# facebookresearch/CPC_audio

Hardware: AMD Instinct MI355X
Metric: audio-seconds/sec (train step) (higher is better)
Workload: dtype f32 (conv GEMMs and the GRU forward recurrence: fp32 operands as 2 scaled fp16 pieces -- the inputs of conv1/conv2 stored that way --, 3 fp16 MFMAs per product; GRU backward recurrence and the criterion's dz gather-GEMM: f32 MFMAs; InfoNCE scores: 2 fp16 pieces; other GEMMs: 3 bf16 pieces, 6 bf16 MF

## Files before the change

cpc_audio_amd/_lib.py:

```python
import ctypes
import os
import threading

_HERE = os.path.dirname(os.path.abspath(__file__))
LIB_PATH = os.path.join(_HERE, "lib", "libcpc_hip.so")
DEFAULT_GRU_MODE = 2
DEFAULT_GRU_XCD_LOCAL = 1
DEFAULT_GRU_POLL_PLAIN = 15
DEFAULT_MFMA_MODE = 3
EXPECTED_ABI = 16
DEFAULT_DMA_PIPELINE = 2
DEFAULT_WGRAD_DMA_STAGES = 4
DEFAULT_CONV_SMALL_PIPE = 1
DEFAULT_GRU_WGRAD_STREAM = 1
DEFAULT_NCE_FUSED = 2
DEFAULT_INDEX_PREP_GROUPS = -1
DEFAULT_FWD_NSPLIT = 0
DEFAULT_DGRAD_NSPLIT = 256
DEFAULT_STEP_SCHEDULE = (1, 0)

_P = ctypes.c_void_p
_I = ctypes.c_int
_L = ctypes.c_long
_F = ctypes.c_float

SIGNATURES = {
    "cpc_abi_version": (_I, []),
    "cpc_release_stream": (_I, [_P]),
    "cpc_streams_overlap": (_I, [_P, _P, _P]),
    "cpc_set_mfma_mode": (_I, [_I]),
    "cpc_get_mfma_mode": (_I, []),
    "cpc_device_error_flags": (_I, [_I]),
    "cpc_conv0_forward": (_I, [_P] * 8 + [_I, _I, _P]),
    "cpc_conv0_forward_h2": (_I, [_P] * 9 + [_I, _I, _P]),
    "cpc_h2_encode": (_I, [_P, _P, _L, _P, _P]),
    "cpc_h2_decode": (_I, [_P, _P, _L, _P, _P]),
    "cpc_conv_weight_relayout_h2": (_I, [_P, _P, _I, _P]),
    "cpc_conv_gemm_forward_h2": (_I, [_P] * 11 + [_I] * 6 + [_P]),
    "cpc_set_dma_tile": (_I, [_I]),
    "cpc_set_conv0_tuning": (_I, [_I, _I]),
# ... 216 lines not shown
```

cpc_audio_amd/csrc/gru.hip:

```cpp
#include "cpc_common.h"
#include "cpc_internal.h"
#include "gemm_tile.h"
#include "persist.h"

namespace cpc {

constexpr int kH = kC;
constexpr int kG = 3 * kH;

__global__ __launch_bounds__(256) void gru_step_fwd_kernel(
    const float* __restrict__ hprev, long hp_bstride, const float* __restrict__ whh,
    const float* __restrict__ bhh, const float* __restrict__ gi, float* __restrict__ y,
    float* __restrict__ Rg, float* __restrict__ Zg, float* __restrict__ Ng, float* __restrict__ GHN,
    float* __restrict__ hN, int B, int S, int t) {
    __shared__ float part[4][3][256];
    const int tid = threadIdx.x, lane = tid & 63, w = tid >> 6;
    const int i = lane & 15, kq = lane >> 4;
    const int j0 = blockIdx.x * 16, b0 = blockIdx.y * 16;
    const int koff = 64 * w + 4 * kq;

    float4 a[4];
    {
        const bool ok = hprev != nullptr && (b0 + i) < B;
        const float* ap = hprev + (ok ? (long)(b0 + i) * hp_bstride + koff : 0);
// ... 218 lines not shown
    if (layer == 0) {
#pragma unroll
        for (int g = 0; g < 3; ++g)
            gh[g] = (((part[0][g][e] + part[1][g][e]) + (part[2][g][e] + part[3][g][e])) +
                     ((part[4][g][e] + part[5][g][e]) + (part[6][g][e] + part[7][g][e]))) + bh[g];
    } else {
#pragma unroll
        for (int g = 0; g < 3; ++g)
            gh[g] = ((part[0][g][e] + part[1][g][e]) + (part[2][g][e] + part[3][g][e])) + bh[g];
        gi_r += (part[4][0][e] + part[5][0][e]) + (part[6][0][e] + part[7][0][e]);
        gi_z += (part[4][1][e] + part[5][1][e]) + (part[6][1][e] + part[7][1][e]);
        gi_n += (part[4][2][e] + part[5][2][e]) + (part[6][2][e] + part[7][2][e]);
    }
    const float r = sigmoidf_(gi_r + gh[0]);
    const float z = sigmoidf_(gi_z + gh[1]);
    const float n = tanhf(gi_n + r * gh[2]);
    const float h = (1.0f - z) * n + z * hp;
    p.y[layer][bt * kH + j] = h;
    p.R[layer][bt * kH + j] = r;
    p.Z[layer][bt * kH + j] = z;
    p.N[layer][bt * kH + j] = n;
    p.GHN[layer][bt * kH + j] = gh[2];
    if (t == S - 1) p.hN[((long)layer * B + b) * kH + j] = h;
}

struct Gru2Bwd {
    const float* dy;
    const float* whhT[2];
    const float* wih1T;
    const float* Z[2];
    const float* cr[2]; const float* cz[2]; const float* cnh[2]; const float* cni[2];
    float* dGi[2]; float* dGh[2]; float* DH[2];
    float* xdh[2];
    int B, S;
    int spin_limit;
    int ntiles, xcd_pack;
    int tile0, total_tiles;
    int first_sleep;
    int poll_plain;
    unsigned* xsync;
};

__global__ __launch_bounds__(256) void gru_bwd_coef_kernel(
    const float* __restrict__ R, const float* __restrict__ Z, const float* __restrict__ N,
    const float* __restrict__ GHN, const float* __restrict__ y, const float* __restrict__ h0,
    float* __restrict__ cr, float* __restrict__ cz, float* __restrict__ cnh, float* __restrict__ cni, int B, int S) {
    const int ntiles = (B + 15) >> 4;
    const long idx = (long)blockIdx.x * 256 + threadIdx.x;
    if (idx >= (long)ntiles * 16 * S * 64) return;
    const int u4 = (int)(idx & 63);
    const long bt = idx >> 6;
    const int b = (int)(bt / S), t = (int)(bt - (long)b * S);
    const long dst = xtile(t, b >> 4, ntiles, kH) + xpos(b & 15, 4 * u4);
    if (b >= B) {
        const float4 zero = make_float4(0.f, 0.f, 0.f, 0.f);
        *reinterpret_cast<float4*>(cr + dst) = zero;
        *reinterpret_cast<float4*>(cz + dst) = zero;
        *reinterpret_cast<float4*>(cnh + dst) = zero;
        *reinterpret_cast<float4*>(cni + dst) = zero;
        return;
    }
    const long src = bt * kH + 4 * u4;
    const float4 r = *reinterpret_cast<const float4*>(R + src), z = *reinterpret_cast<const float4*>(Z + src);
    const float4 n = *reinterpret_cast<const float4*>(N + src), g = *reinterpret_cast<const float4*>(GHN + src);
    float4 hp = make_float4(0.f, 0.f, 0.f, 0.f);
    if (t > 0) hp = *reinterpret_cast<const float4*>(y + src - kH);
// ... 77 lines not shown
        }
    } else if (w < 4) {
        if (has_next) {
            const float* grow = p.dGh[0] + (bok ? ((long)(b0 + i) * S + t + 1) * kG : 0);
            acc = mfma_gate_rows<4>(acc, grow, bok, p.whhT[0] + (long)(j0 + i) * kG, 64 * w + 4 * kq);
        }
    } else {
        const float* grow = p.dGi[1] + (bok ? ((long)(b0 + i) * S + t) * kG : 0);
        acc = mfma_gate_rows<4>(acc, grow, bok, p.wih1T + (long)(j0 + i) * kG, 64 * (w - 4) + 4 * kq);
    }
#pragma unroll
    for (int rr = 0; rr < 4; ++rr) part[w][(kq * 4 + rr) * 16 + i] = acc[rr];
    __syncthreads();
    if (!gate_thread) return;
    const int e = tid;
    const float dh = (((part[0][e] + part[1][e]) + (part[2][e] + part[3][e])) +
                      ((part[4][e] + part[5][e]) + (part[6][e] + part[7][e]))) + dh0;
    float* gi = p.dGi[layer] + bt * kG;
    float* gh = p.dGh[layer] + bt * kG;
    const float dar = dh * cr, daz = dh * cz;
    gi[j] = dar;            gh[j] = dar;
    gi[kH + j] = daz;       gh[kH + j] = daz;
    gi[2 * kH + j] = dh * cni;   gh[2 * kH + j] = dh * cnh;
    p.DH[layer][bt * kH + j] = dh;
}

constexpr int kSpinLimit = 1 << 20;
static __device__ unsigned g_gru_poll_timeout = 0;

__device__ __forceinline__ void store_handover(float* p, float v, bool local) {
    if (local) __hip_atomic_store(p, v, __ATOMIC_RELAXED, __HIP_MEMORY_SCOPE_WAVEFRONT);
    else __hip_atomic_store(p, v, __ATOMIC_RELAXED, __HIP_MEMORY_SCOPE_AGENT);
}
__device__ __forceinline__ bool tile_on_one_xcd(unsigned* sync, int spin_limit) {
    __shared__ unsigned verdict;
    if (threadIdx.x == 0) {
        const unsigned xid = __builtin_amdgcn_s_getreg((3 << 11) | 20) & 15u;
        __hip_atomic_fetch_and(sync, ~(1u << xid), __ATOMIC_RELAXED, __HIP_MEMORY_SCOPE_AGENT);
        __hip_atomic_fetch_add(sync + 1, 1u, __ATOMIC_RELEASE, __HIP_MEMORY_SCOPE_AGENT);
        int budget = spin_limit < 4096 ? spin_limit : 4096;
        while (__hip_atomic_load(sync + 1, __ATOMIC_ACQUIRE, __HIP_MEMORY_SCOPE_AGENT) != 31u && budget-- > 0) __builtin_amdgcn_s_sleep(8);
        const unsigned gone = ~__hip_atomic_load(sync, __ATOMIC_RELAXED, __HIP_MEMORY_SCOPE_AGENT);
        verdict = (budget > 0 && gone != 0u && (gone & (gone - 1u)) == 0u) ? 1u : 0u;
    }
    __syncthreads();
    return verdict != 0u;
}

template <int NII>
__device__ __forceinline__ void poll_row(const float* __restrict__ row, bool ok, float4 (&a)[NII], int& budget,
                                         PollPace& pace, bool plain_first = false) {
    poll_frags<NII, kXStride>(row, ok, a, budget, pace, &g_gru_poll_timeout, plain_first);
}

template <int NII>
__device__ __forceinline__ void load_row_plain(const float* __restrict__ row, bool ok, float4 (&a)[NII]) {
#pragma unroll
    for (int ii = 0; ii < NII; ++ii)
        a[ii] = ok ? *reinterpret_cast<const float4*>(row + 16 * ii) : make_float4(0.f, 0.f, 0.f, 0.f);
}

template <int NII>
__device__ __forceinline__ void load_gate_weights(float4 (&bw)[3][NII], const float* __restrict__ w, int j0i, int koff) {
#pragma unroll
    for (int g = 0; g < 3; ++g)
#pragma unroll
        for (int ii = 0; ii < NII; ++ii)
            bw[g][ii] = *reinterpret_cast<const float4*>(w + (long)(g * kH + j0i) * kH + koff + 16 * ii);
}

template <int NII>
__device__ __forceinline__ void mfma_gates(f32x4 (&acc)[3], const float4 (&a)[NII], const float4 (&bw)[3][NII]) {
#pragma unroll
    for (int ii = 0; ii < NII; ++ii)
// ... 50 lines not shown
__device__ unsigned long long g_gru_phase[2][512][12][8];
struct PhaseClock {
    unsigned long long last, sum[8];
    __device__ PhaseClock() : last(0) { for (int i = 0; i < 8; ++i) sum[i] = 0; }
    __device__ __forceinline__ void start() {
        __builtin_amdgcn_sched_barrier(0);
        last = __builtin_readcyclecounter();
        __builtin_amdgcn_sched_barrier(0);
    }
    __device__ __forceinline__ void lap(int i, bool on) {
        __builtin_amdgcn_sched_barrier(0);
        const unsigned long long now = __builtin_readcyclecounter();
        if (on) sum[i] += now - last;
        last = now;
        __builtin_amdgcn_sched_barrier(0);
    }
    __device__ __forceinline__ void flush(int dir) {
        if ((threadIdx.x & 63) == 0 && blockIdx.x < 512)
            for (int i = 0; i < 8; ++i) g_gru_phase[dir][blockIdx.x][threadIdx.x >> 6][i] = sum[i];
    }
};
#else
struct PhaseClock {
    __device__ __forceinline__ void start() {}
    __device__ __forceinline__ void lap(int, bool) {}
    __device__ __forceinline__ void flush(int) {}
};
#endif

struct PersistIds {
    int layer, j0, b0, tile, ntiles, G;
    bool valid;
    __device__ PersistIds(int G, int pack, int tile0, int total) {
        int rest;
        if (pack) {
            const int xcd = blockIdx.x & 7, slot = blockIdx.x >> 3;
            tile = (slot >> 5) * 8 + xcd;
            rest = slot & 31;
        } else {
            tile = blockIdx.x % G;
            rest = blockIdx.x / G;
        }
        valid = tile < G && tile0 + tile < total;
        tile += tile0;
        ntiles = total;
        this->G = G;
        b0 = tile * 16;
        layer = rest >> 4;
        j0 = (rest & 15) * 16;
    }
};

constexpr int kPersistThreads = 768;
constexpr int kMfmaWaves = 8;

template <int LAYER, bool H2, int NT>
__device__ __forceinline__ void persist_fwd(const Gru2Fwd& p, float (&part)[2][8][3][256], const PersistIds& id, bool local) {
    const int j0 = id.j0;
    constexpr int NII = LAYER == 0 ? 2 : 4;
    const int tid = threadIdx.x, lane = tid & 63, w = tid >> 6;
    const int B = p.B, S = p.S;
    float* __restrict__ yl = p.y[LAYER];
    int tl[NT];
#pragma unroll
    for (int k = 0; k < NT; ++k) tl[k] = id.tile + k * id.G;

    if (w < kMfmaWaves) {
        const int i = lane & 15, kq = lane >> 4;
        const bool recurrent = LAYER == 0 || w < 4;
        const int koff = LAYER == 0 ? 32 * w + 4 * kq : 64 * (w & 3) + 4 * kq;
        float4 bw[3][NII];
        load_gate_weights<NII>(bw, recurrent ? p.whh[LAYER] : p.wih1, j0 + i, koff);
        H2Frag bh[3][NII / 2];
        float sa = 1.f, inv = 1.f;
        if constexpr (H2) {
// ... 115 lines not shown
            const float h = (1.0f - z) * n + z * hp[k];
            store_handover(p.xh[LAYER] + xtile(t, tl[k], id.ntiles, kH) + xpos(e >> 4, j), h, local);
            pc.lap(4, traced);
            yl[bt * kH + j] = h;
            p.R[LAYER][bt * kH + j] = r;
            p.Z[LAYER][bt * kH + j] = z;
            p.N[LAYER][bt * kH + j] = n;
            p.GHN[LAYER][bt * kH + j] = gh[2];
            if (t == S - 1) p.hN[((long)LAYER * B + b[k]) * kH + j] = h;
            if (cf) {
                const float a = (1.0f - z) * (1.0f - n * n);
                const long c = xtile(t, tl[k], id.ntiles, kH) + cpos;
                cf[c] = a * gh[2] * r * (1.0f - r);
                cf[c + p.frag_stride] = (hp[k] - n) * z * (1.0f - z);
                cf[c + 2 * p.frag_stride] = a * r;
                cf[c + 3 * p.frag_stride] = a;
            }
            hp[k] = h;
            if (LAYER == 0 && t + 1 < S) {
                const float* gip = p.x_gi0 + (bt + 1) * kG;
                gi[k][0] = gip[j]; gi[k][1] = gip[kH + j]; gi[k][2] = gip[2 * kH + j];
            }
            pc.lap(5, traced);
        }
    }
    pc.flush(0);
}

template <int NT>
__global__ __launch_bounds__(kPersistThreads) void gru2_persist_fwd_kernel(Gru2Fwd p) {
    __shared__ float part[2][8][3][256];
    const PersistIds id(p.ntiles, p.xcd_pack, p.tile0, p.total_tiles);
    if (!id.valid) return;
    const bool local = p.xsync != nullptr && tile_on_one_xcd(p.xsync + 2 * id.tile, p.spin_limit);
    if (id.layer == 0) persist_fwd<0, false, NT>(p, part, id, local);
    else persist_fwd<1, false, NT>(p, part, id, local);
}
template <int NT>
__global__ __launch_bounds__(kPersistThreads) void gru2_persist_fwd_h2_kernel(Gru2Fwd p) {
    __shared__ float part[2][8][3][256];
    const PersistIds id(p.ntiles, p.xcd_pack, p.tile0, p.total_tiles);
    if (!id.valid) return;
    const bool local = p.xsync != nullptr && tile_on_one_xcd(p.xsync + 2 * id.tile, p.spin_limit);
    if (id.layer == 0) persist_fwd<0, true, NT>(p, part, id, local);
    else persist_fwd<1, true, NT>(p, part, id, local);
}

template <int NU>
__device__ __forceinline__ void load_coef(float4 (&cf)[NU][3], const float* __restrict__ c0, const float* __restrict__ c1,
                                          const float* __restrict__ c2, long off) {
#pragma unroll
    for (int ii = 0; ii < NU; ++ii) {
        cf[ii][0] = *reinterpret_cast<const float4*>(c0 + off + kXStride * ii);
        cf[ii][1] = *reinterpret_cast<const float4*>(c1 + off + kXStride * ii);
        cf[ii][2] = *reinterpret_cast<const float4*>(c2 + off + kXStride * ii);
    }
}

template <int LAYER, int NT>
__device__ __forceinline__ void persist_bwd(const Gru2Bwd& p, float (&part)[2][8][256], const PersistIds& id, bool local) {
    constexpr int NU = LAYER == 1 ? 2 : 4;
    const int j0 = id.j0;
    const int tid = threadIdx.x, lane = tid & 63, w = tid >> 6;
    const int B = p.B, S = p.S;
    int tl[NT];
#pragma unroll
    for (int k = 0; k < NT; ++k) tl[k] = id.tile + k * id.G;

    if (w < kMfmaWaves) {
        const int i = lane & 15, kq = lane >> 4;
        const bool recurrent = LAYER == 1 || w < 4;
        const int unit0 = LAYER == 1 ? 32 * w + 4 * kq : 64 * (w & 3) + 4 * kq;
        float4 bw[NU][3];
        {
            const float* wrow = (recurrent ? p.whhT[LAYER] : p.wih1T) + (long)(j0 + i) * kG;
#pragma unroll
            for (int ii = 0; ii < NU; ++ii)
#pragma unroll
                for (int g = 0; g < 3; ++g)
                    bw[ii][g] = *reinterpret_cast<const float4*>(wrow + g * kH + unit0 + 16 * ii);
        }
        const int sl = recurrent ? LAYER : 1;
        const float* __restrict__ c0 = p.cr[sl];
        const float* __restrict__ c1 = p.cz[sl];
        const float* __restrict__ c2 = recurrent ? p.cnh[sl] : p.cni[sl];
        const long lane_off = xpos(i, unit0);
        const float* __restrict__ xsrc = p.xdh[sl] + lane_off;
        bool tok[NT], bok[NT];
#pragma unroll
        for (int k = 0; k < NT; ++k) {
            tok[k] = tl[k] < id.ntiles;
            bok[k] = tok[k] && (tl[k] * 16 + i) < B;
        }
        float4 cf[NU][3];
        if (NT == 1 && !recurrent) load_coef<NU>(cf, c0, c1, c2, xtile(S - 1, tl[0], id.ntiles, kH) + lane_off);
        int budget = p.spin_limit;
        PollPace pace(p.first_sleep);
        PhaseClock pc;
        pc.start();
        for (int t = S - 1; t >= 0; --t) {
            const int ts = recurrent ? t + 1 : t;
            const bool traced = t >= 16 && t < S - 16;
#pragma unroll
            for (int k = 0; k < NT; ++k) {
                f32x4 acc = f32x4{0.f, 0.f, 0.f, 0.f};
                if (ts < S && tok[k]) {
                    if (NT > 1) load_coef<NU>(cf, c0, c1, c2, xtile(ts, tl[k], id.ntiles, kH) + lane_off);
                    float4 dh[NU];
                    poll_row<NU>(xsrc + xtile(ts, tl[k], id.ntiles, kH), bok[k], dh, budget, pace,
                                 (p.poll_plain & (recurrent ? 8 : 2)) != 0);
                    pc.lap(0, traced);
                    f32x4 ag[3];
#pragma unroll
                    for (int g = 0; g < 3; ++g) ag[g] = f32x4{0.f, 0.f, 0.f, 0.f};
#pragma unroll
                    for (int hf = 0; hf < 2; ++hf) {
                        float4 op[NU / 2][3];
#pragma unroll
                        for (int ii = 0; ii < NU / 2; ++ii)
#pragma unroll
// ... 36 lines not shown
    float dyv[NT], z[NT], cr[NT], cz[NT], cnh[NT], cni[NT];
    float dh_next[NT], z_next[NT];
    auto fetch = [&](int k, int t) __attribute__((always_inline)) {
        const long bt = (long)b[k] * S + t;
        if (LAYER == 1) dyv[k] = p.dy[bt * kH + j];
        z[k] = p.Z[LAYER][bt * kH + j];
        const long c = xtile(t, tl[k], id.ntiles, kH) + xp;
        cr[k] = p.cr[LAYER][c]; cz[k] = p.cz[LAYER][c]; cnh[k] = p.cnh[LAYER][c]; cni[k] = p.cni[LAYER][c];
    };
#pragma unroll
    for (int k = 0; k < NT; ++k) {
        b[k] = tl[k] * 16 + row;
        live[k] = tl[k] < id.ntiles && b[k] < B;
        dyv[k] = z[k] = cr[k] = cz[k] = cnh[k] = cni[k] = 0.f;
        dh_next[k] = z_next[k] = 0.f;
        if (live[k]) fetch(k, S - 1);
    }
    PhaseClock pc;
    pc.start();
    for (int t = S - 1; t >= 0; --t) {
        const bool traced = t >= 16 && t < S - 16;
#pragma unroll
        for (int k = 0; k < NT; ++k) {
            __syncthreads();
            pc.lap(3, traced);
            if (!live[k]) continue;
            const long bt = (long)b[k] * S + t;
            float (&pt)[8][256] = part[(t * NT + k) & 1];
            float dh0 = LAYER == 1 ? dyv[k] : 0.f;
            if ((t + 1) < S) dh0 = fmaf(dh_next[k], z_next[k], dh0);
            const float dh = (((pt[0][e] + pt[1][e]) + (pt[2][e] + pt[3][e])) +
                              ((pt[4][e] + pt[5][e]) + (pt[6][e] + pt[7][e]))) + dh0;
            store_handover(p.xdh[LAYER] + xtile(t, tl[k], id.ntiles, kH) + xp, dh, local);
            pc.lap(4, traced);
            float* gi = p.dGi[LAYER] + bt * kG;
            float* gh = p.dGh[LAYER] + bt * kG;
            const float dar = dh * cr[k], daz = dh * cz[k];
            __builtin_nontemporal_store(dar, gi + j); __builtin_nontemporal_store(dar, gh + j);
            __builtin_nontemporal_store(daz, gi + kH + j); __builtin_nontemporal_store(daz, gh + kH + j);
            __builtin_nontemporal_store(dh * cni[k], gi + 2 * kH + j); __builtin_nontemporal_store(dh * cnh[k], gh + 2 * kH + j);
            __builtin_nontemporal_store(dh, p.DH[LAYER] + bt * kH + j);
            dh_next[k] = dh;
            z_next[k] = z[k];
            if (t > 0) fetch(k, t - 1);
            pc.lap(5, traced);
        }
    }
    pc.flush(1);
}

template <int NT>
__global__ __launch_bounds__(kPersistThreads) void gru2_persist_bwd_kernel(Gru2Bwd p) {
    __shared__ float part[2][8][256];
    const PersistIds id(p.ntiles, p.xcd_pack, p.tile0, p.total_tiles);
    if (!id.valid) return;
    const bool local = p.xsync != nullptr && tile_on_one_xcd(p.xsync + 2 * id.tile, p.spin_limit);
    if (id.layer == 0) persist_bwd<1, NT>(p, part, id, local);
    else persist_bwd<0, NT>(p, part, id, local);
}

struct GruLayout {
    long R[8], Z[8], N[8], GHN[8], Y[8];
    long saved_total;
    long gi, xh, xh_floats, fwd_total;
    long whhT, wihT, dGi, dGh, DH, mid[2], part, tmp;
    long whhT2, wihT2, dGi2, dGh2, DH2;
    long coef, xdh, frag_floats;
    long sync_floats;
    long bwd_total;
};

static bool gru_layout(int B, int S, int nl, GruLayout& g) {
    if (B <= 0 || S <= 0 || nl <= 0 || nl > 8) return false;
    const long bsh = align64l((long)B * S * kH);
    long o = 0;
    for (int l = 0; l < nl; ++l) {
        g.R[l] = o; o += bsh;
        g.Z[l] = o; o += bsh;
        g.N[l] = o; o += bsh;
        g.GHN[l] = o; o += bsh;
        g.Y[l] = -1;
        if (l < nl - 1) { g.Y[l] = o; o += bsh; }
    }
    g.saved_total = o;
    const long tiles16 = (long)cdiv(B, 16) * 16;
    g.gi = 0;
    g.xh = align64l((long)B * S * kG);
    g.xh_floats = nl == 2 ? align64l((long)S * tiles16 * kH) : 0;
    g.sync_floats = nl == 2 ? align64l(2L * cdiv(B, 16)) : 0;
    g.fwd_total = g.xh + 2 * g.xh_floats + g.sync_floats;
    o = 0;
    g.whhT = o; o += (long)kH * kG;
    g.wihT = o; o += (long)kH * kG;
    g.dGi = o; o += align64l((long)B * S * kG);
    g.dGh = o; o += align64l((long)B * S * kG);
    g.DH = o; o += bsh;
    g.mid[0] = o; o += bsh;
    g.mid[1] = o; o += bsh;
    g.part = o; o += align64l(std::max(tn_gemm_part_floats(B * S, kG, kH), tn_gemm_batch_part_floats(4, B * S, kG, kH)));
    g.tmp = o; o += 4 * align64l((long)kRowsSumGroups * kG);
    g.whhT2 = o; o += (long)kH * kG;
    g.wihT2 = o; o += (long)kH * kG;
    g.dGi2 = o; o += align64l((long)B * S * kG);
    g.dGh2 = o; o += align64l((long)B * S * kG);
    g.DH2 = o; o += bsh;
    g.frag_floats = nl == 2 ? align64l((long)S * tiles16 * kH) : 0;
    g.coef = o; o += 8 * g.frag_floats;
    g.xdh = o; o += 2 * g.frag_floats + g.sync_floats;
    g.bwd_total = o;
    return true;
}

}

using namespace cpc;

namespace {
int g_gru_spin_limit = kSpinLimit;
int g_gru_first_sleep[2] = {-1, -1};
int g_gru_poll_plain = 15;
int g_gru_xcd_local = 1;
int g_gru_xcd_pack = 0;
int g_gru_mode = 2;

int g_gru_chunk_tiles = 0;
static int persist_chunk(const void* kernel, int G) {
    int dev = 0, cus = 0, occ = 0;
    if (hipGetDevice(&dev) != hipSuccess) return 0;
    if (hipDeviceGetAttribute(&cus, hipDeviceAttributeMultiprocessorCount, dev) != hipSuccess) return 0;
    if (hipOccupancyMaxActiveBlocksPerMultiprocessor(&occ, kernel, kPersistThreads, 0) != hipSuccess) return 0;
    int fit = (int)(((long)cus * occ) / 32);
    if (g_gru_chunk_tiles > 0 && fit > g_gru_chunk_tiles) fit = g_gru_chunk_tiles;
    return fit >= G ? G : fit;
}

int g_gru_tiles_per_wg = 2;
static void persist_plan(int total, int fit1, int fit2, int* G, int* NT) {
    if (fit1 >= total || g_gru_tiles_per_wg < 2 || fit2 <= 0) { *G = fit1 >= total ? total : fit1; *NT = 1; return; }
    const int slots = (total + 1) / 2;
    *G = slots < fit2 ? slots : fit2;
    *NT = 2;
}

static bool xcd_local_wanted(int dirbit, int NT) {
    if (g_gru_xcd_local & (4 << dirbit)) return true;
    return (g_gru_xcd_local & (1 << dirbit)) && NT == 1;
}
template <class K>
int persist_grid(K kernel, int G, int* pack, bool want_pack = false) {
    int dev = 0, cus = 0, occ = 0;
    *pack = 0;
    if (hipGetDevice(&dev) != hipSuccess) return 0;
    if (hipDeviceGetAttribute(&cus, hipDeviceAttributeMultiprocessorCount, dev) != hipSuccess) return 0;
    if (hipOccupancyMaxActiveBlocksPerMultiprocessor(&occ, kernel, kPersistThreads, 0) != hipSuccess) return 0;
    const long room = (long)cus * occ;
    if (32L * G > room) return 0;
    if (g_gru_xcd_pack == 2 || ((g_gru_xcd_pack == 1 || want_pack) && cus % 8 == 0 && 32L * cdiv(G, 8) <= (long)(cus / 8) * occ)) {
        *pack = 1;
        return 256 * cdiv(G, 8);
    }
    return 32 * G;
}
}

namespace cpc {
int gru_error_flag_fetch(int clear, unsigned* out) { return device_flag_fetch(HIP_SYMBOL(g_gru_poll_timeout), clear, out); }
}

extern "C" int cpc_set_gru_spin_limit(int limit) {
    g_gru_spin_limit = limit < 0 ? kSpinLimit : limit;
    return 0;
}

extern "C" int cpc_set_gru_poll_pacing(int first_fwd, int first_bwd) {
    if (first_fwd > 200 || first_bwd > 200 || first_fwd < -255 || first_bwd < -255) return CPC_ERR_ARG;
    g_gru_first_sleep[0] = first_fwd;
    g_gru_first_sleep[1] = first_bwd;
    return 0;
}

extern "C" int cpc_set_gru_chunk_tiles(int tiles) {
    if (tiles < 0) return CPC_ERR_ARG;
    g_gru_chunk_tiles = tiles;
    return 0;
}

extern "C" int cpc_set_gru_tiles_per_wg(int n) {
    if (n != 1 && n != 2) return CPC_ERR_ARG;
    g_gru_tiles_per_wg = n;
    return 0;
}

extern "C" int cpc_set_gru_poll_plain(int mask) {
    if (mask < 0 || mask > 31) return CPC_ERR_ARG;
// ... 59 lines not shown
    hipStream_t st = (hipStream_t)stream;
    const float* in = x;
    float* gi = scratch + g.gi;
    if (nl == 2) {
        int rc = nt_gemm(plain_rows(x, B * S, kH), params[0], kH, params[2], gi, kG, kG, kH, st);
        if (rc) return rc;
        Gru2Fwd p;
        p.x_gi0 = gi;
        for (int l = 0; l < 2; ++l) {
            p.h0[l] = h0 ? h0 + (long)l * B * kH : nullptr;
            p.whh[l] = params[4 * l + 1];
            p.bhh[l] = params[4 * l + 3];
            p.R[l] = saved + g.R[l]; p.Z[l] = saved + g.Z[l]; p.N[l] = saved + g.N[l]; p.GHN[l] = saved + g.GHN[l];
        }
        p.wih1 = params[4]; p.bih1 = params[6];
        p.y[0] = saved + g.Y[0]; p.y[1] = y;
        p.hN = hN; p.B = B; p.S = S; p.spin_limit = g_gru_spin_limit;
        p.first_sleep = g_gru_first_sleep[0];
        p.poll_plain = g_gru_poll_plain;
        p.xh[0] = p.xh[1] = nullptr;
        p.xsync = nullptr;
        p.coef[0] = p.coef[1] = nullptr;
        p.frag_stride = g.frag_floats;
        p.total_tiles = cdiv(B, 16);
        p.tile0 = 0;
        const bool h2 = g_gru_mode == 2 && !h0;
        int NT = 1;
        {
            const int fit1 = persist_chunk(h2 ? (const void*)gru2_persist_fwd_h2_kernel<1> : (const void*)gru2_persist_fwd_kernel<1>, p.total_tiles);
            const int fit2 = persist_chunk(h2 ? (const void*)gru2_persist_fwd_h2_kernel<2> : (const void*)gru2_persist_fwd_kernel<2>, p.total_tiles);
            persist_plan(p.total_tiles, fit1, fit2, &p.ntiles, &NT);
        }
        const int nblocks = g_gru_mode < 1 || p.ntiles <= 0 ? 0
                            : h2 ? (NT == 2 ? persist_grid(gru2_persist_fwd_h2_kernel<2>, p.ntiles, &p.xcd_pack, xcd_local_wanted(0, NT))
                                            : persist_grid(gru2_persist_fwd_h2_kernel<1>, p.ntiles, &p.xcd_pack, xcd_local_wanted(0, NT)))
                                 : (NT == 2 ? persist_grid(gru2_persist_fwd_kernel<2>, p.ntiles, &p.xcd_pack, xcd_local_wanted(0, NT))
                                            : persist_grid(gru2_persist_fwd_kernel<1>, p.ntiles, &p.xcd_pack, xcd_local_wanted(0, NT)));
        if (nblocks > 0) {
            p.xh[0] = scratch + g.xh; p.xh[1] = scratch + g.xh + g.xh_floats;
            if (coef) { p.coef[0] = coef; p.coef[1] = coef + 4 * g.frag_floats; }
            if (!xh_ready && hipMemsetAsync(p.xh[0], 0xFF, (2 * g.xh_floats + g.sync_floats) * sizeof(float), st) != hipSuccess) return CPC_ERR_ARG;
            p.xsync = xcd_local_wanted(0, NT) && p.xcd_pack ? reinterpret_cast<unsigned*>(scratch + g.xh + 2 * g.xh_floats) : nullptr;
            step_timer_mark(3, st);
            for (p.tile0 = 0; p.tile0 < p.total_tiles; p.tile0 += p.ntiles * NT) {
                if (h2 && NT == 2) hipLaunchKernelGGL(gru2_persist_fwd_h2_kernel<2>, dim3(nblocks), dim3(kPersistThreads), 0, st, p);
                else if (h2) hipLaunchKernelGGL(gru2_persist_fwd_h2_kernel<1>, dim3(nblocks), dim3(kPersistThreads), 0, st, p);
                else if (NT == 2) hipLaunchKernelGGL(gru2_persist_fwd_kernel<2>, dim3(nblocks), dim3(kPersistThreads), 0, st, p);
                else hipLaunchKernelGGL(gru2_persist_fwd_kernel<1>, dim3(nblocks), dim3(kPersistThreads), 0, st, p);
            }
            step_timer_mark(4, st);
            CPC_LAUNCH_CHECK();
            return 0;
        }
        const dim3 grid(kH / 16, cdiv(B, 16), 2);
        for (int s = 0; s <= S; ++s) hipLaunchKernelGGL(gru2_fwd_kernel, grid, dim3(512), 0, st, p, s);
        if (coef) launch_gru_coef(g, h0, saved, y, coef, B, S, st);
        CPC_LAUNCH_CHECK();
        return 0;
    }
    for (int l = 0; l < nl; ++l) {
        const float* wih = params[4 * l], *whh = params[4 * l + 1], *bih = params[4 * l + 2], *bhh = params[4 * l + 3];
        float* out = (l == nl - 1) ? y : saved + g.Y[l];
        int rc = nt_gemm(plain_rows(in, B * S, kH), wih, kH, bih, gi, kG, kG, kH, st);
        if (rc) return rc;
        const float* h0l = h0 ? h0 + (long)l * B * kH : nullptr;
        const dim3 grid(kH / 16, cdiv(B, 16));
        for (int t = 0; t < S; ++t) {
            const float* hprev = t == 0 ? h0l : out + (long)(t - 1) * kH;
            const long hstride = t == 0 ? kH : (long)S * kH;
            hipLaunchKernelGGL(gru_step_fwd_kernel, grid, dim3(256), 0, st, hprev, hstride, whh, bhh, gi, out,
                               saved + g.R[l], saved + g.Z[l], saved + g.N[l], saved + g.GHN[l],
                               t == S - 1 ? hN + (long)l * B * kH : nullptr, B, S, t);
        }
        CPC_LAUNCH_CHECK();
        in = out;
    }
    return 0;
}

extern "C" long cpc_gru_coef_floats(int B, int S, int nl) {
    GruLayout g;
    if (nl != 2 || !gru_layout(B, S, nl, g)) return 0;
    return 10 * g.frag_floats + g.sync_floats + 4L * kG * kH;
}

static void launch_gru_coef(const GruLayout& g, const float* h0, const float* saved, const float* y, float* coef,
                            int B, int S, hipStream_t st) {
    const float* yl[2] = {saved + g.Y[0], y};
    const float* h0l[2] = {h0, h0 ? h0 + (long)B * kH : nullptr};
    for (int l = 0; l < 2; ++l) {
        float* c = coef + 4 * l * g.frag_floats;
        hipLaunchKernelGGL(gru_bwd_coef_kernel, dim3(cdiv((long)cdiv(B, 16) * 16 * S * 64, 256)), dim3(256), 0, st,
                           saved + g.R[l], saved + g.Z[l], saved + g.N[l], saved + g.GHN[l], yl[l], h0l[l], c,
                           c + g.frag_floats, c + 2 * g.frag_floats, c + 3 * g.frag_floats, B, S);
    }
}

extern "C" int cpc_gru_backward_coef(const float* h0, const float* const* params, const float* saved, const float* y,
                                     float* coef, int coef_done, int B, int S, int nl, void* stream) {
    GruLayout g;
    CPC_RETURN_IF(nl != 2 || !gru_layout(B, S, nl, g), CPC_ERR_SHAPE);
    CPC_RETURN_IF(!params || !saved || !y || !coef, CPC_ERR_ARG);
    if (!coef_done) launch_gru_coef(g, h0, saved, y, coef, B, S, (hipStream_t)stream);
    {
        float* wT = coef + 10 * g.frag_floats + g.sync_floats;
        const float* tin[4] = {params[1], params[0], params[5], params[4]};
        float* tout[4] = {wT, wT + (long)kG * kH, wT + 2L * kG * kH, wT + 3L * kG * kH};
        int rc = transpose_batch(tin, tout, 4, kG, kH, (hipStream_t)stream);
        if (rc) return rc;
    }
    if (hipMemsetAsync(coef + 8 * g.frag_floats, 0xFF, (2 * g.frag_floats + g.sync_floats) * sizeof(float), (hipStream_t)stream) != hipSuccess)
        return CPC_ERR_ARG;
    CPC_LAUNCH_CHECK();
    return 0;
}

extern "C" int cpc_gru_backward(const float* x, const float* h0, const float* const* params,
                                const float* saved, const float* y, const float* dy, float* scratch,
                                float* dx, float* const* grads, int B, int S, int nl, void* stream) {
    return cpc_gru_backward_with_coef(x, h0, params, saved, y, dy, nullptr, scratch, dx, grads, B, S, nl, stream);
}

extern "C" int cpc_gru_backward_with_coef(const float* x, const float* h0, const float* const* params,
                                          const float* saved, const float* y, const float* dy, const float* coef,
                                          float* scratch, float* dx, float* const* grads, int B, int S, int nl,
                                          void* stream) {
    return cpc_gru_backward_streams(x, h0, params, saved, y, dy, coef, scratch, dx, grads, B, S, nl, stream, stream);
}

extern "C" int cpc_gru_backward_streams(const float* x, const float* h0, const float* const* params,
                                        const float* saved, const float* y, const float* dy, const float* coef,
                                        float* scratch, float* dx, float* const* grads, int B, int S, int nl,
                                        void* stream, void* wgrad_stream) {
    GruLayout g;
    CPC_RETURN_IF(!gru_layout(B, S, nl, g), CPC_ERR_SHAPE);
    CPC_RETURN_IF(!x || !params || !saved || !scratch || !y || !dy || !dx || !grads, CPC_ERR_ARG);
    hipStream_t st = (hipStream_t)stream;
    hipStream_t wst = nl == 2 ? (hipStream_t)wgrad_stream : st;
    float* whhT = scratch + g.whhT, *wihT = scratch + g.wihT;
    float* dGi = scratch + g.dGi, *dGh = scratch + g.dGh, *DH = scratch + g.DH;
    const int M = B * S;
    if (nl == 2) {
        float* cwT = coef ? const_cast<float*>(coef) + 10 * g.frag_floats + g.sync_floats : nullptr;
        float* whhT_[2] = {coef ? cwT : scratch + g.whhT, coef ? cwT + 2L * kG * kH : scratch + g.whhT2};
        float* wihT_[2] = {coef ? cwT + (long)kG * kH : scratch + g.wihT, coef ? cwT + 3L * kG * kH : scratch + g.wihT2};
        float* dGi_[2] = {scratch + g.dGi, scratch + g.dGi2};
        float* dGh_[2] = {scratch + g.dGh, scratch + g.dGh2};
        float* DH_[2] = {scratch + g.DH, scratch + g.DH2};
        Gru2Bwd p;
        p.dy = dy; p.B = B; p.S = S; p.spin_limit = g_gru_spin_limit;
        p.first_sleep = g_gru_first_sleep[1];
        p.poll_plain = g_gru_poll_plain;
        const float* yl[2] = {saved + g.Y[0], y};
        const float* h0l[2] = {h0, h0 ? h0 + (long)B * kH : nullptr};
        int rc = 0;
        if (!coef) {
            const float* tin[4] = {params[1], params[0], params[5], params[4]};
            float* tout[4] = {whhT_[0], wihT_[0], whhT_[1], wihT_[1]};
            rc = transpose_batch(tin, tout, 4, kG, kH, st);
            if (rc) return rc;
        }
        for (int l = 0; l < 2; ++l) {
            p.whhT[l] = whhT_[l];
            p.Z[l] = saved + g.Z[l];
            p.dGi[l] = dGi_[l]; p.dGh[l] = dGh_[l]; p.DH[l] = DH_[l];
            const float* c = (coef ? coef : scratch + g.coef) + 4 * l * g.frag_floats;
            p.cr[l] = c; p.cz[l] = c + g.frag_floats; p.cnh[l] = c + 2 * g.frag_floats; p.cni[l] = c + 3 * g.frag_floats;
            p.xdh[l] = (coef ? const_cast<float*>(coef) + 8 * g.frag_floats : scratch + g.xdh) + l * g.frag_floats;
        }
        if (!coef) launch_gru_coef(g, h0, saved, y, scratch + g.coef, B, S, st);
        p.wih1T = wihT_[1];
        p.xsync = nullptr;
        p.total_tiles = cdiv(B, 16);
        p.tile0 = 0;
        int NT = 1;
        persist_plan(p.total_tiles, persist_chunk((const void*)gru2_persist_bwd_kernel<1>, p.total_tiles),
                     persist_chunk((const void*)gru2_persist_bwd_kernel<2>, p.total_tiles), &p.ntiles, &NT);
        if (NT == 2 && !(g_gru_poll_plain & 16)) p.poll_plain = 0;
        const int nblocks = g_gru_mode < 1 || p.ntiles <= 0 ? 0
                            : NT == 2 ? persist_grid(gru2_persist_bwd_kernel<2>, p.ntiles, &p.xcd_pack, xcd_local_wanted(1, NT))
                                      : persist_grid(gru2_persist_bwd_kernel<1>, p.ntiles, &p.xcd_pack, xcd_local_wanted(1, NT));
        if (nblocks > 0) {
            if (!coef && hipMemsetAsync(p.xdh[0], 0xFF, (2 * g.frag_floats + g.sync_floats) * sizeof(float), st) != hipSuccess) return CPC_ERR_ARG;
            p.xsync = xcd_local_wanted(1, NT) && p.xcd_pack ? reinterpret_cast<unsigned*>(p.xdh[0] + 2 * g.frag_floats) : nullptr;
            for (p.tile0 = 0; p.tile0 < p.total_tiles; p.tile0 += p.ntiles * NT) {
                if (NT == 2) hipLaunchKernelGGL(gru2_persist_bwd_kernel<2>, dim3(nblocks), dim3(kPersistThreads), 0, st, p);
                else hipLaunchKernelGGL(gru2_persist_bwd_kernel<1>, dim3(nblocks), dim3(kPersistThreads), 0, st, p);
            }
            step_timer_mark(6, st);
        } else {
            const dim3 grid(kH / 16, cdiv(B, 16), 2);
            for (int s = 0; s <= S; ++s) hipLaunchKernelGGL(gru2_bwd_kernel, grid, dim3(512), 0, st, p, s);
        }
        CPC_LAUNCH_CHECK();
        SplitK sk;
        sk.part = scratch + g.part;
        sk.floats = std::max(tn_gemm_part_floats(B * S, kG, kH), tn_gemm_batch_part_floats(4, B * S, kG, kH));
        rc = nt_gemm(plain_rows(dGi_[0], M, kG), wihT_[0], kG, nullptr, dx, kH, kH, kG, st, 0, 0, GemmBounds(), GemmGroup(), sk);
        if (rc) return rc;
        if (wst != st) {
            hipEvent_t* ev = stream_events(st);
            CPC_RETURN_IF(!ev, CPC_ERR_ARG);
            if (hipEventRecord(ev[8], st) != hipSuccess || hipStreamWaitEvent(wst, ev[8], 0) != hipSuccess) return CPC_ERR_ARG;
        }
        const long tmp1 = align64l((long)kRowsSumGroups * kG);
        const RowsSumJob jobs[4] = {{dGi_[0], M, kG, scratch + g.tmp, grads[2]},
                                    {dGh_[0], M, kG, scratch + g.tmp + tmp1, grads[3]},
                                    {dGi_[1], M, kG, scratch + g.tmp + 2 * tmp1, grads[6]},
                                    {dGh_[1], M, kG, scratch + g.tmp + 3 * tmp1, grads[7]}};
        {
            RowMap am[4], bm[4];
            float* Cq[4];
            for (int l = 0; l < 2; ++l) {
                const float* in = l == 0 ? x : saved + g.Y[0];
                am[2 * l] = plain_rows(dGi_[l], M, kG);
                bm[2 * l] = plain_rows(in, M, kH);
                Cq[2 * l] = grads[4 * l];
// ... 71 lines not shown
```

cpc_audio_amd/csrc/persist.h:

```cpp
#pragma once
#include "cpc_common.h"

namespace cpc {

constexpr unsigned kNotReady = 0xFFFFFFFFu;

__device__ __forceinline__ float4 load4_coherent(const float* p) {
    const unsigned long long* q = reinterpret_cast<const unsigned long long*>(p);
    const unsigned long long lo = __hip_atomic_load(q, __ATOMIC_RELAXED, __HIP_MEMORY_SCOPE_AGENT);
    const unsigned long long hi = __hip_atomic_load(q + 1, __ATOMIC_RELAXED, __HIP_MEMORY_SCOPE_AGENT);
    return make_float4(__uint_as_float((unsigned)lo), __uint_as_float((unsigned)(lo >> 32)),
                       __uint_as_float((unsigned)hi), __uint_as_float((unsigned)(hi >> 32)));
}
__device__ __forceinline__ float4 load4_plain(const float* p) {
    const unsigned long long* q = reinterpret_cast<const unsigned long long*>(p);
    const unsigned long long lo = __hip_atomic_load(q, __ATOMIC_RELAXED, __HIP_MEMORY_SCOPE_WAVEFRONT);
    const unsigned long long hi = __hip_atomic_load(q + 1, __ATOMIC_RELAXED, __HIP_MEMORY_SCOPE_WAVEFRONT);
    return make_float4(__uint_as_float((unsigned)lo), __uint_as_float((unsigned)(lo >> 32)),
                       __uint_as_float((unsigned)hi), __uint_as_float((unsigned)(hi >> 32)));
}
__device__ __forceinline__ bool ready4(float4 v) {
    return __float_as_uint(v.x) != kNotReady && __float_as_uint(v.y) != kNotReady &&
           __float_as_uint(v.z) != kNotReady && __float_as_uint(v.w) != kNotReady;
}
// ... 18 lines not shown

template <int NII, int STRIDE>
__device__ __forceinline__ void poll_frags(const float* __restrict__ row, bool ok, float4 (&a)[NII], int& budget,
                                           PollPace& pace, unsigned* timeout_flag, bool plain_first = false) {
    for (int q = 0; q < pace.delay; ++q) __builtin_amdgcn_s_sleep(1);
    if (plain_first) {
#pragma unroll
        for (int ii = 0; ii < NII; ++ii) a[ii] = load4_plain(row + STRIDE * ii);
    } else {
#pragma unroll
        for (int ii = 0; ii < NII; ++ii) a[ii] = load4_coherent(row + STRIDE * ii);
    }
    int repeats = 0;
    for (;;) {
        bool rdy = true;
#pragma unroll
        for (int ii = 0; ii < NII; ++ii) rdy = rdy && ready4(a[ii]);
        if (__all(rdy || !ok) || budget <= 0) break;
        --budget;
        ++repeats;
        __builtin_amdgcn_s_sleep(1);
#pragma unroll
        for (int ii = 0; ii < NII; ++ii)
            if (ok && !ready4(a[ii])) a[ii] = load4_coherent(row + STRIDE * ii);
    }
    pace.update(repeats);
    if (budget <= 0) atomicOr(timeout_flag, 1u);
    if (!ok) {
#pragma unroll
        for (int ii = 0; ii < NII; ++ii) a[ii] = make_float4(0.f, 0.f, 0.f, 0.f);
    }
}

}
```

Measured before the change: 31320.

## Pack GRU backward persistent blocks per layer group onto one XCD

```diff
diff --git a/cpc_audio_amd/_lib.py b/cpc_audio_amd/_lib.py
--- a/cpc_audio_amd/_lib.py
+++ b/cpc_audio_amd/_lib.py
@@ -5,7 +5,7 @@
 _HERE = os.path.dirname(os.path.abspath(__file__))
 LIB_PATH = os.path.join(_HERE, "lib", "libcpc_hip.so")
 DEFAULT_GRU_MODE = 2
-DEFAULT_GRU_XCD_LOCAL = 1
+DEFAULT_GRU_XCD_LOCAL = 3
 DEFAULT_GRU_POLL_PLAIN = 15
 DEFAULT_MFMA_MODE = 3
 EXPECTED_ABI = 16
diff --git a/cpc_audio_amd/csrc/gru.hip b/cpc_audio_amd/csrc/gru.hip
--- a/cpc_audio_amd/csrc/gru.hip
+++ b/cpc_audio_amd/csrc/gru.hip
@@ -274,6 +274,7 @@
     const float* cr[2]; const float* cz[2]; const float* cnh[2]; const float* cni[2];
     float* dGi[2]; float* dGh[2]; float* DH[2];
     float* xdh[2];
+    float* xdh1r;
     int B, S;
     int spin_limit;
     int ntiles, xcd_pack;
@@ -417,14 +418,23 @@
     if (local) __hip_atomic_store(p, v, __ATOMIC_RELAXED, __HIP_MEMORY_SCOPE_WAVEFRONT);
     else __hip_atomic_store(p, v, __ATOMIC_RELAXED, __HIP_MEMORY_SCOPE_AGENT);
 }
-__device__ __forceinline__ bool tile_on_one_xcd(unsigned* sync, int spin_limit) {
+__device__ __forceinline__ unsigned xcc_id() {
+#ifdef HIPEMU
+    const char* e = getenv("HIPEMU_XCDS");
+    const int n = e ? atoi(e) : 0;
+    return n > 1 ? (unsigned)(blockIdx.x % (unsigned)n) & 15u : 0u;
+#else
+    return __builtin_amdgcn_s_getreg((3 << 11) | 20) & 15u;
+#endif
+}
+__device__ __forceinline__ bool on_one_xcd(unsigned* sync, int spin_limit, unsigned members) {
     __shared__ unsigned verdict;
     if (threadIdx.x == 0) {
-        const unsigned xid = __builtin_amdgcn_s_getreg((3 << 11) | 20) & 15u;
+        const unsigned xid = xcc_id();
         __hip_atomic_fetch_and(sync, ~(1u << xid), __ATOMIC_RELAXED, __HIP_MEMORY_SCOPE_AGENT);
         __hip_atomic_fetch_add(sync + 1, 1u, __ATOMIC_RELEASE, __HIP_MEMORY_SCOPE_AGENT);
         int budget = spin_limit < 4096 ? spin_limit : 4096;
-        while (__hip_atomic_load(sync + 1, __ATOMIC_ACQUIRE, __HIP_MEMORY_SCOPE_AGENT) != 31u && budget-- > 0) __builtin_amdgcn_s_sleep(8);
+        while (__hip_atomic_load(sync + 1, __ATOMIC_ACQUIRE, __HIP_MEMORY_SCOPE_AGENT) != members - 1u && budget-- > 0) __builtin_amdgcn_s_sleep(8);
         const unsigned gone = ~__hip_atomic_load(sync, __ATOMIC_RELAXED, __HIP_MEMORY_SCOPE_AGENT);
         verdict = (budget > 0 && gone != 0u && (gone & (gone - 1u)) == 0u) ? 1u : 0u;
     }
@@ -541,15 +551,9 @@
     int layer, j0, b0, tile, ntiles, G;
     bool valid;
     __device__ PersistIds(int G, int pack, int tile0, int total) {
-        int rest;
-        if (pack) {
-            const int xcd = blockIdx.x & 7, slot = blockIdx.x >> 3;
-            tile = (slot >> 5) * 8 + xcd;
-            rest = slot & 31;
-        } else {
-            tile = blockIdx.x % G;
-            rest = blockIdx.x / G;
-        }
+        const PersistSlot s = persist_slot((int)blockIdx.x, G, pack);
+        const int rest = s.rest;
+        tile = s.tile;
         valid = tile < G && tile0 + tile < total;
         tile += tile0;
         ntiles = total;
@@ -731,7 +735,7 @@
     __shared__ float part[2][8][3][256];
     const PersistIds id(p.ntiles, p.xcd_pack, p.tile0, p.total_tiles);
     if (!id.valid) return;
-    const bool local = p.xsync != nullptr && tile_on_one_xcd(p.xsync + 2 * id.tile, p.spin_limit);
+    const bool local = p.xsync != nullptr && on_one_xcd(p.xsync + 4 * id.tile, p.spin_limit, 32u);
     if (id.layer == 0) persist_fwd<0, false, NT>(p, part, id, local);
     else persist_fwd<1, false, NT>(p, part, id, local);
 }
@@ -740,7 +744,7 @@
     __shared__ float part[2][8][3][256];
     const PersistIds id(p.ntiles, p.xcd_pack, p.tile0, p.total_tiles);
     if (!id.valid) return;
-    const bool local = p.xsync != nullptr && tile_on_one_xcd(p.xsync + 2 * id.tile, p.spin_limit);
+    const bool local = p.xsync != nullptr && on_one_xcd(p.xsync + 4 * id.tile, p.spin_limit, 32u);
     if (id.layer == 0) persist_fwd<0, true, NT>(p, part, id, local);
     else persist_fwd<1, true, NT>(p, part, id, local);
 }
@@ -784,7 +788,7 @@
         const float* __restrict__ c1 = p.cz[sl];
         const float* __restrict__ c2 = recurrent ? p.cnh[sl] : p.cni[sl];
         const long lane_off = xpos(i, unit0);
-        const float* __restrict__ xsrc = p.xdh[sl] + lane_off;
+        const float* __restrict__ xsrc = (!recurrent && p.xdh1r ? p.xdh1r : p.xdh[sl]) + lane_off;
         bool tok[NT], bok[NT];
 #pragma unroll
         for (int k = 0; k < NT; ++k) {
@@ -887,6 +891,7 @@
             const float dh = (((pt[0][e] + pt[1][e]) + (pt[2][e] + pt[3][e])) +
                               ((pt[4][e] + pt[5][e]) + (pt[6][e] + pt[7][e]))) + dh0;
             store_handover(p.xdh[LAYER] + xtile(t, tl[k], id.ntiles, kH) + xp, dh, local);
+            if (LAYER == 1 && p.xdh1r) store_coherent(p.xdh1r + xtile(t, tl[k], id.ntiles, kH) + xp, dh);
             pc.lap(4, traced);
             float* gi = p.dGi[LAYER] + bt * kG;
             float* gh = p.dGh[LAYER] + bt * kG;
@@ -909,7 +914,8 @@
     __shared__ float part[2][8][256];
     const PersistIds id(p.ntiles, p.xcd_pack, p.tile0, p.total_tiles);
     if (!id.valid) return;
-    const bool local = p.xsync != nullptr && tile_on_one_xcd(p.xsync + 2 * id.tile, p.spin_limit);
+    const bool group = p.xcd_pack == kPackGroup;
+    const bool local = p.xsync != nullptr && on_one_xcd(p.xsync + 4 * id.tile + (group ? 2 * id.layer : 0), p.spin_limit, group ? 16u : 32u);
     if (id.layer == 0) persist_bwd<1, NT>(p, part, id, local);
     else persist_bwd<0, NT>(p, part, id, local);
 }
@@ -924,6 +930,9 @@
     long sync_floats;
     long bwd_total;
 };
+
+constexpr int kXdhBufs = 3;
+constexpr int kCoefBufs = 8 + kXdhBufs;
 
 static bool gru_layout(int B, int S, int nl, GruLayout& g) {
     if (B <= 0 || S <= 0 || nl <= 0 || nl > 8) return false;
@@ -942,7 +951,7 @@
     g.gi = 0;
     g.xh = align64l((long)B * S * kG);
     g.xh_floats = nl == 2 ? align64l((long)S * tiles16 * kH) : 0;
-    g.sync_floats = nl == 2 ? align64l(2L * cdiv(B, 16)) : 0;
+    g.sync_floats = nl == 2 ? align64l(4L * cdiv(B, 16)) : 0;
     g.fwd_total = g.xh + 2 * g.xh_floats + g.sync_floats;
     o = 0;
     g.whhT = o; o += (long)kH * kG;
@@ -961,7 +970,7 @@
     g.DH2 = o; o += bsh;
     g.frag_floats = nl == 2 ? align64l((long)S * tiles16 * kH) : 0;
     g.coef = o; o += 8 * g.frag_floats;
-    g.xdh = o; o += 2 * g.frag_floats + g.sync_floats;
+    g.xdh = o; o += kXdhBufs * g.frag_floats + g.sync_floats;
     g.bwd_total = o;
     return true;
 }
@@ -974,7 +983,7 @@
 int g_gru_spin_limit = kSpinLimit;
 int g_gru_first_sleep[2] = {-1, -1};
 int g_gru_poll_plain = 15;
-int g_gru_xcd_local = 1;
+int g_gru_xcd_local = 3;
 int g_gru_xcd_pack = 0;
 int g_gru_mode = 2;
 
@@ -1001,20 +1010,21 @@
     if (g_gru_xcd_local & (4 << dirbit)) return true;
     return (g_gru_xcd_local & (1 << dirbit)) && NT == 1;
 }
+static int bwd_pack_wanted(int NT) {
+    if (NT == 1 && (g_gru_xcd_local & (2 | 8))) return kPackGroup;
+    return (g_gru_xcd_local & 8) ? kPackTile : kPackNone;
+}
 template <class K>
-int persist_grid(K kernel, int G, int* pack, bool want_pack = false) {
+int persist_grid(K kernel, int G, int* pack, int want = kPackNone) {
     int dev = 0, cus = 0, occ = 0;
-    *pack = 0;
+    *pack = kPackNone;
     if (hipGetDevice(&dev) != hipSuccess) return 0;
     if (hipDeviceGetAttribute(&cus, hipDeviceAttributeMultiprocessorCount, dev) != hipSuccess) return 0;
     if (hipOccupancyMaxActiveBlocksPerMultiprocessor(&occ, kernel, kPersistThreads, 0) != hipSuccess) return 0;
-    const long room = (long)cus * occ;
-    if (32L * G > room) return 0;
-    if (g_gru_xcd_pack == 2 || ((g_gru_xcd_pack == 1 || want_pack) && cus % 8 == 0 && 32L * cdiv(G, 8) <= (long)(cus / 8) * occ)) {
-        *pack = 1;
-        return 256 * cdiv(G, 8);
-    }
-    return 32 * G;
+    if (!persist_pack_fits(G, kPackNone, cus, occ)) return 0;
+    if (want == kPackNone && g_gru_xcd_pack >= 1) want = kPackTile;
+    if (want != kPackNone && (g_gru_xcd_pack == 2 || persist_pack_fits(G, want, cus, occ))) *pack = want;
+    return persist_grid_size(G, *pack);
 }
 }
 
@@ -1140,10 +1150,10 @@
             persist_plan(p.total_tiles, fit1, fit2, &p.ntiles, &NT);
         }
         const int nblocks = g_gru_mode < 1 || p.ntiles <= 0 ? 0
-                            : h2 ? (NT == 2 ? persist_grid(gru2_persist_fwd_h2_kernel<2>, p.ntiles, &p.xcd_pack, xcd_local_wanted(0, NT))
-                                            : persist_grid(gru2_persist_fwd_h2_kernel<1>, p.ntiles, &p.xcd_pack, xcd_local_wanted(0, NT)))
-                                 : (NT == 2 ? persist_grid(gru2_persist_fwd_kernel<2>, p.ntiles, &p.xcd_pack, xcd_local_wanted(0, NT))
-                                            : persist_grid(gru2_persist_fwd_kernel<1>, p.ntiles, &p.xcd_pack, xcd_local_wanted(0, NT)));
+                            : h2 ? (NT == 2 ? persist_grid(gru2_persist_fwd_h2_kernel<2>, p.ntiles, &p.xcd_pack, xcd_local_wanted(0, NT) ? kPackTile : kPackNone)
+                                            : persist_grid(gru2_persist_fwd_h2_kernel<1>, p.ntiles, &p.xcd_pack, xcd_local_wanted(0, NT) ? kPackTile : kPackNone))
+                                 : (NT == 2 ? persist_grid(gru2_persist_fwd_kernel<2>, p.ntiles, &p.xcd_pack, xcd_local_wanted(0, NT) ? kPackTile : kPackNone)
+                                            : persist_grid(gru2_persist_fwd_kernel<1>, p.ntiles, &p.xcd_pack, xcd_local_wanted(0, NT) ? kPackTile : kPackNone));
         if (nblocks > 0) {
             p.xh[0] = scratch + g.xh; p.xh[1] = scratch + g.xh + g.xh_floats;
             if (coef) { p.coef[0] = coef; p.coef[1] = coef + 4 * g.frag_floats; }
@@ -1189,7 +1199,7 @@
 extern "C" long cpc_gru_coef_floats(int B, int S, int nl) {
     GruLayout g;
     if (nl != 2 || !gru_layout(B, S, nl, g)) return 0;
-    return 10 * g.frag_floats + g.sync_floats + 4L * kG * kH;
+    return kCoefBufs * g.frag_floats + g.sync_floats + 4L * kG * kH;
 }
 
 static void launch_gru_coef(const GruLayout& g, const float* h0, const float* saved, const float* y, float* coef,
@@ -1211,13 +1221,13 @@
     CPC_RETURN_IF(!params || !saved || !y || !coef, CPC_ERR_ARG);
     if (!coef_done) launch_gru_coef(g, h0, saved, y, coef, B, S, (hipStream_t)stream);
     {
-        float* wT = coef + 10 * g.frag_floats + g.sync_floats;
+        float* wT = coef + kCoefBufs * g.frag_floats + g.sync_floats;
         const float* tin[4] = {params[1], params[0], params[5], params[4]};
         float* tout[4] = {wT, wT + (long)kG * kH, wT + 2L * kG * kH, wT + 3L * kG * kH};
         int rc = transpose_batch(tin, tout, 4, kG, kH, (hipStream_t)stream);
         if (rc) return rc;
     }
-    if (hipMemsetAsync(coef + 8 * g.frag_floats, 0xFF, (2 * g.frag_floats + g.sync_floats) * sizeof(float), (hipStream_t)stream) != hipSuccess)
+    if (hipMemsetAsync(coef + 8 * g.frag_floats, 0xFF, (kXdhBufs * g.frag_floats + g.sync_floats) * sizeof(float), (hipStream_t)stream) != hipSuccess)
         return CPC_ERR_ARG;
     CPC_LAUNCH_CHECK();
     return 0;
@@ -1249,7 +1259,7 @@
     float* dGi = scratch + g.dGi, *dGh = scratch + g.dGh, *DH = scratch + g.DH;
     const int M = B * S;
     if (nl == 2) {
-        float* cwT = coef ? const_cast<float*>(coef) + 10 * g.frag_floats + g.sync_floats : nullptr;
+        float* cwT = coef ? const_cast<float*>(coef) + kCoefBufs * g.frag_floats + g.sync_floats : nullptr;
         float* whhT_[2] = {coef ? cwT : scratch + g.whhT, coef ? cwT + 2L * kG * kH : scratch + g.whhT2};
         float* wihT_[2] = {coef ? cwT + (long)kG * kH : scratch + g.wihT, coef ? cwT + 3L * kG * kH : scratch + g.wihT2};
         float* dGi_[2] = {scratch + g.dGi, scratch + g.dGi2};
@@ -1279,6 +1289,7 @@
         if (!coef) launch_gru_coef(g, h0, saved, y, scratch + g.coef, B, S, st);
         p.wih1T = wihT_[1];
         p.xsync = nullptr;
+        p.xdh1r = nullptr;
         p.total_tiles = cdiv(B, 16);
         p.tile0 = 0;
         int NT = 1;
@@ -1286,11 +1297,12 @@
                      persist_chunk((const void*)gru2_persist_bwd_kernel<2>, p.total_tiles), &p.ntiles, &NT);
         if (NT == 2 && !(g_gru_poll_plain & 16)) p.poll_plain = 0;
         const int nblocks = g_gru_mode < 1 || p.ntiles <= 0 ? 0
-                            : NT == 2 ? persist_grid(gru2_persist_bwd_kernel<2>, p.ntiles, &p.xcd_pack, xcd_local_wanted(1, NT))
-                                      : persist_grid(gru2_persist_bwd_kernel<1>, p.ntiles, &p.xcd_pack, xcd_local_wanted(1, NT));
+                            : NT == 2 ? persist_grid(gru2_persist_bwd_kernel<2>, p.ntiles, &p.xcd_pack, bwd_pack_wanted(NT))
+                                      : persist_grid(gru2_persist_bwd_kernel<1>, p.ntiles, &p.xcd_pack, bwd_pack_wanted(NT));
         if (nblocks > 0) {
-            if (!coef && hipMemsetAsync(p.xdh[0], 0xFF, (2 * g.frag_floats + g.sync_floats) * sizeof(float), st) != hipSuccess) return CPC_ERR_ARG;
-            p.xsync = xcd_local_wanted(1, NT) && p.xcd_pack ? reinterpret_cast<unsigned*>(p.xdh[0] + 2 * g.frag_floats) : nullptr;
+            if (!coef && hipMemsetAsync(p.xdh[0], 0xFF, (kXdhBufs * g.frag_floats + g.sync_floats) * sizeof(float), st) != hipSuccess) return CPC_ERR_ARG;
+            p.xsync = bwd_pack_wanted(NT) && p.xcd_pack ? reinterpret_cast<unsigned*>(p.xdh[0] + kXdhBufs * g.frag_floats) : nullptr;
+            if (p.xcd_pack == kPackGroup) p.xdh1r = p.xdh[0] + 2 * g.frag_floats;
             for (p.tile0 = 0; p.tile0 < p.total_tiles; p.tile0 += p.ntiles * NT) {
                 if (NT == 2) hipLaunchKernelGGL(gru2_persist_bwd_kernel<2>, dim3(nblocks), dim3(kPersistThreads), 0, st, p);
                 else hipLaunchKernelGGL(gru2_persist_bwd_kernel<1>, dim3(nblocks), dim3(kPersistThreads), 0, st, p);
diff --git a/cpc_audio_amd/csrc/persist.h b/cpc_audio_amd/csrc/persist.h
--- a/cpc_audio_amd/csrc/persist.h
+++ b/cpc_audio_amd/csrc/persist.h
@@ -74,4 +74,31 @@
     }
 }
 
+constexpr int kPackNone = 0, kPackTile = 1, kPackGroup = 2;
+struct PersistSlot { int tile, rest; };
+__host__ __device__ inline PersistSlot persist_slot(int bid, int G, int pack) {
+    PersistSlot s;
+    const int xcd = bid & 7, slot = bid >> 3;
+    if (pack == kPackGroup) {
+        const int group = (slot >> 4) * 8 + xcd;
+        s.tile = group >> 1;
+        s.rest = (group & 1) * 16 + (slot & 15);
+    } else if (pack == kPackTile) {
+        s.tile = (slot >> 5) * 8 + xcd;
+        s.rest = slot & 31;
+    } else {
+        s.tile = bid % G;
+        s.rest = bid / G;
+    }
+    return s;
 }
+__host__ __device__ inline int persist_grid_size(int G, int pack) {
+    return pack == kPackGroup ? 128 * ((2 * G + 7) / 8) : pack == kPackTile ? 256 * ((G + 7) / 8) : 32 * G;
+}
+__host__ __device__ inline bool persist_pack_fits(int G, int pack, int cus, int occ) {
+    if (pack == kPackNone) return 32L * G <= (long)cus * occ;
+    if (cus <= 0 || cus % 8 != 0) return false;
+    return (long)(persist_grid_size(G, pack) / 8) <= (long)(cus / 8) * occ;
+}
+
+}
```

New measurement: 31850 (median of 6 runs). +1.7%, better.
